# D-Robotics/hobot_stereonet

Hardware: AMD Instinct MI355X
Metric: stereo pairs/s at 1280x720 D=192 (ms/frame alongside) (higher is better)
Workload: dtype f16 (refinement-tower MFMA operands fp16 — 3x3 weights rounded per kernel so that every kernel's tap sum survives —, LeakyReLU applied after the fp16 rounding; low-resolution branch on 22-bit hi/lo split fp16 operands, 3 fp16 MFMAs per product in every 32-channel layer — profiles/r04_lowres_ablation

## Files before the change

hobot_stereonet_amd/csrc/sn_kernels.hpp:

```cpp
#pragma once
#include <hip/hip_runtime.h>
#include <stdint.h>

#include <type_traits>

#ifndef SN_X3S_FPK
#define SN_X3S_FPK 2
#endif
#ifndef SN_X3S_WAGPR
#define SN_X3S_WAGPR 1
#endif

namespace sn {

typedef float f32x16 __attribute__((ext_vector_type(16)));
typedef float f32x4 __attribute__((ext_vector_type(4)));

typedef _Float16 half8 __attribute__((ext_vector_type(8)));
typedef _Float16 half4 __attribute__((ext_vector_type(4)));

constexpr int kC = 32;
constexpr int kRefPad = 8;
constexpr float kSplitScale = 2048.0f;
constexpr float kSplitInv = 1.0f / 2048.0f;
// ... 1481 lines not shown
    if (NBUF == 3) {
      more = g0 + 3 < G;
      if (more) issue(g0 + 3, nimg_, ny0, nx0);
    } else {
      more = g0 + 2 < G;
      if (more) issue(g0 + 2, nimg_, ny0, nx0);
    }
    compute(lds + ((g0 + 1) % NBUF) * RING, std::integral_constant<int, 1>{}, acc0, acc1);
    if (RES) {
      if (more) wait_vmcnt<KW2>(); else wait_vmcnt<0>();
#pragma unroll
      for (int i = 0; i < 2 * T::NSTORE; ++i) asm volatile("" : "+v"(rres[i]));
    }
    const bool interior = y0 + T::TH <= g.H && x0 + T::TW <= g.W;
#pragma unroll
    for (int q = 0; q < 4; ++q) {
      char* oq = reinterpret_cast<char*>(out) + (tb + (unsigned)q * plane_b);
      char* oql = out_lo + (tb + (unsigned)q * plane_b);
#pragma unroll
      for (int s = 0; s < T::SPW; ++s) {
        half4 hh, hl;
#pragma unroll
        for (int e = 0; e < 4; ++e) {
          float v = acc0[s][4 * q + e] + acc1[s][4 * q + e] * kSplitInv;
          if (RES) {
            const uint2 rh = rres[RES ? 2 * (s * 4 + q) : 0], rl = rres[RES ? 2 * (s * 4 + q) + 1 : 0];
            const half4 vh = *reinterpret_cast<const half4*>(&rh);
            const half4 vl = *reinterpret_cast<const half4*>(&rl);
            v += (float)vh[e] + (float)vl[e] * kSplitInv;
          }
          if (lrelu) v = lrelu_fast(v);
          const _Float16 hi = (_Float16)v;
          hh[e] = hi;
          hl[e] = (_Float16)((v - (float)hi) * kSplitScale);
        }
        if (!interior) {
          const int seg = seg0 + s;
          const int y = y0 + seg / T::CSEG, x = x0 + (seg % T::CSEG) * 32 + j;
          if (!(y < g.H && x < g.W)) {
            hh = half4{(_Float16)0.f, (_Float16)0.f, (_Float16)0.f, (_Float16)0.f};
            hl = hh;
          }
        }
        *reinterpret_cast<half4*>(oq + io_voff[s]) = hh;
        *reinterpret_cast<half4*>(oql + io_voff[s]) = hl;
      }
    }
    img = nimg_;
    y0 = ny0;
    x0 = nx0;
  }
}

template <int TW_>
struct RefInTile {
  static constexpr int TH = 8, TW = TW_, CSEG = TW / 32;
  static constexpr int ROWS = TH + 2, COLS = TW + 8;
  static constexpr int BUF = ROWS * COLS;
  static constexpr int LDS_BYTES = 2 * BUF * 16;
  static constexpr int NUNIT = ROWS * (COLS / 4);
  static constexpr int SPW = TH * CSEG / 4;
};

template <bool SPLIT, bool PYR, int TW>
__global__ __launch_bounds__(256, 2) void k_refin_f16(const float* __restrict__ disp_low,
                                                   const void* __restrict__ img_src,
                                                   int hl, int wl, int H, int W, float inv_d, UpScale ups,
                                                   const uint4* __restrict__ wfrag,
                                                   const float* __restrict__ bias, uint4* __restrict__ out,
                                                   size_t lo_off_bytes, RefGeom g, int nimg, int al4) {
  using T = RefInTile<TW>;
  static_assert(T::NUNIT <= 256, "one staging unit per thread");
  extern __shared__ __attribute__((aligned(16))) uint4 s_px[];
  const int tid = threadIdx.x, lane = tid & 63;
  const int wave = __builtin_amdgcn_readfirstlane(tid >> 6);
  const int j = lane & 31, gk = lane >> 5;

  half8 wa[5], wb[5];
#pragma unroll
  for (int t = 0; t < 5; ++t) {
    const uint4 a = wfrag[(2 * t) * 64 + lane], b = wfrag[(2 * t + 1) * 64 + lane];
    wa[t] = *reinterpret_cast<const half8*>(&a);
    wb[t] = *reinterpret_cast<const half8*>(&b);
  }
  f32x16 bv;
#pragma unroll
  for (int r = 0; r < 16; ++r) bv[r] = bias[(r & 3) + 8 * (r >> 2) + 4 * gk];
  int koff[5];
#pragma unroll
  for (int t = 0; t < 5; ++t) {
    int tap = 2 * t + gk;
    tap = tap < 9 ? tap : 0;
    koff[t] = (tap / 3) * T::COLS + (tap % 3) + 3;
  }

  const int per_img = g.tiles_x * g.tiles_y;
  const int total = per_img * nimg;
  const int ur = tid / (T::COLS / 4), uq = tid - ur * (T::COLS / 4);
  const bool unit = tid < T::NUNIT;
  const int8_t* const in6 = reinterpret_cast<const int8_t*>(img_src);
  const float* const pyr = reinterpret_cast<const float*>(img_src);
  const bool x16 = ups.rs == 1.0f / 16.0f;
  uint32_t pimg[3];
  float pf[PYR ? 3 : 1][4];
  float pd[4];
  bool pval[4];
  auto fetch = [&](int tile) {
    if (g.rev) tile = total - 1 - tile;
    const int img = tile / per_img, rem = tile - img * per_img;
    const int ty = rem / g.tiles_x, tx = rem - ty * g.tiles_x;
    const int y = ty * T::TH - 1 + ur, x = tx * T::TW - 4 + 4 * uq;
    pimg[0] = pimg[1] = pimg[2] = 0;
#pragma unroll
    for (int k = 0; k < 4; ++k) {
      pd[k] = 0.f;
      pval[k] = false;
    }
// ... 23 lines not shown
      for (int k = 0; k < 4; ++k)
        if (pval[k]) pd[k] = upsample_map(dl, hl, wl, y, x + k, ups) * inv_d;
    }
    if (PYR) {
#pragma unroll
      for (int c = 0; c < 3; ++c) {
        const float* row = pyr + (((size_t)img * 3 + c) * g.H + y) * (size_t)g.W;
#pragma unroll
        for (int k = 0; k < 4; ++k) pf[PYR ? c : 0][k] = pval[k] ? row[x + k] : 0.f;
      }
    } else if (y < H) {
#pragma unroll
      for (int c = 0; c < 3; ++c) {
        const int8_t* row = in6 + (((size_t)img * 6 + c) * H + y) * (size_t)W;
        uint32_t v = 0;
        if (al4) {
          if (x >= 0 && x + 3 < W) v = *reinterpret_cast<const uint32_t*>(row + x);
        } else {
#pragma unroll
          for (int k = 0; k < 4; ++k)
            if ((unsigned)(x + k) < (unsigned)W) v |= (uint32_t)(uint8_t)row[x + k] << (8 * k);
        }
        pimg[c] = v;
      }
    }
  };
  auto commit = [&](uint4* buf) {
    if (!unit) return;
#pragma unroll
    for (int k = 0; k < 4; ++k) {
      half8 sl;
#pragma unroll
      for (int e = 0; e < 8; ++e) sl[e] = (_Float16)0.f;
      if (pval[k]) {
        const _Float16 dh = (_Float16)pd[k];
        sl[0] = dh;
        sl[4] = (_Float16)((pd[k] - (float)dh) * kSplitScale);
        if (PYR) {
#pragma unroll
          for (int c = 0; c < 3; ++c) {
            const float v = pf[PYR ? c : 0][k];
            const _Float16 vh = (_Float16)v;
            sl[1 + c] = vh;
            sl[5 + c] = (_Float16)((v - (float)vh) * kSplitScale);
          }
        } else {
#pragma unroll
          for (int c = 0; c < 3; ++c) sl[1 + c] = (_Float16)((float)(int8_t)(pimg[c] >> (8 * k)) * (1.0f / 128.0f));
        }
      }
      buf[ur * T::COLS + 4 * uq + k] = *reinterpret_cast<const uint4*>(&sl);
    }
  };

  int tile = blockIdx.x;
  if (tile >= total) return;
  fetch(tile);
  commit(s_px);
  __syncthreads();
  int cur = 0;
  const unsigned plane_b = (unsigned)g.Hs * (unsigned)g.Ws * 16u;
  unsigned io_voff[T::SPW];
#pragma unroll
  for (int s = 0; s < T::SPW; ++s) {
    const int seg = wave * T::SPW + s;
    io_voff[s] = ((unsigned)(seg / T::CSEG) * (unsigned)g.Ws + (unsigned)((seg % T::CSEG) * 32 + j)) * 16u + gk * 8u;
  }
  for (; tile < total; tile += gridDim.x) {
    const int nxt = tile + gridDim.x;
    if (nxt < total) fetch(nxt);
    const uint4* buf = s_px + cur * T::BUF;
    f32x16 acc0[T::SPW], acc1[T::SPW];
    f32x16 zero;
#pragma unroll
    for (int r = 0; r < 16; ++r) zero[r] = 0.f;
#pragma unroll
    for (int t = 0; t < 5; ++t) {
#pragma unroll
      for (int s = 0; s < T::SPW; ++s) {
        const int seg = wave * T::SPW + s;
        const int srow = seg / T::CSEG, scol = (seg % T::CSEG) * 32;
        const uint4 xv = buf[koff[t] + srow * T::COLS + scol + j];
        const half8 xb = *reinterpret_cast<const half8*>(&xv);
        acc0[s] = __builtin_amdgcn_mfma_f32_32x32x16_f16(wa[t], xb, t == 0 ? bv : acc0[s], 0, 0, 0);
        acc1[s] = __builtin_amdgcn_mfma_f32_32x32x16_f16(wb[t], xb, t == 0 ? zero : acc1[s], 0, 0, 0);
      }
    }
    {
      const int tile_m = g.rev ? total - 1 - tile : tile;
      const int img = tile_m / per_img, rem = tile_m - img * per_img;
      const int ty = rem / g.tiles_x, tx = rem - ty * g.tiles_x;
      const int y0 = ty * T::TH, x0 = tx * T::TW;
      const bool interior = y0 + T::TH <= g.H && x0 + T::TW <= g.W;
      const unsigned tb = (((unsigned)img * 4u * (unsigned)g.Hs + (unsigned)(y0 + kRefPad)) * (unsigned)g.Ws +
                           (unsigned)(x0 + kRefPad)) * 16u;
#pragma unroll
      for (int s = 0; s < T::SPW; ++s) {
#pragma unroll
        for (int q = 0; q < 4; ++q) {
          char* oq = reinterpret_cast<char*>(out) + (tb + (unsigned)q * plane_b);
          char* oql = oq + lo_off_bytes;
          half4 hh, hl4;
          if (SPLIT) {
#pragma unroll
            for (int e = 0; e < 4; ++e) {
              float v = acc0[s][4 * q + e] + acc1[s][4 * q + e] * kSplitInv;
              v = lrelu_fast(v);
              const _Float16 hi = (_Float16)v;
              hh[e] = hi;
              hl4[e] = (_Float16)((v - (float)hi) * kSplitScale);
            }
          } else {
            float v[4];
#pragma unroll
            for (int e = 0; e < 4; ++e) v[e] = acc0[s][4 * q + e] + acc1[s][4 * q + e] * kSplitInv;
            const uint2 pk{act_pack2_f16(v[0], v[1], (_Float16)kSlope), act_pack2_f16(v[2], v[3], (_Float16)kSlope)};
            hh = *reinterpret_cast<const half4*>(&pk);
          }
          bool ok = true;
          if (!interior) {
            const int seg = wave * T::SPW + s;
            ok = y0 + seg / T::CSEG < g.H && x0 + (seg % T::CSEG) * 32 + j < g.W;
          }
          if (ok) {
            *reinterpret_cast<half4*>(oq + io_voff[s]) = hh;
            if (SPLIT) *reinterpret_cast<half4*>(oql + io_voff[s]) = hl4;
          }
        }
      }
    }
    if (nxt < total) commit(s_px + (cur ^ 1) * T::BUF);
    lds_barrier();
    cur ^= 1;
  }
}

template <int TH_>
struct HeadTile {
  static constexpr int TH = TH_, TWO = 62;
  static constexpr int RP = TH + 2, CP = 64;
  static constexpr int NSEG = RP * 2, SPW = (NSEG + 3) / 4;
  static constexpr int PLANE = RP * CP;
  static constexpr int LDS_BYTES = 9 * PLANE * 4;
};

template <bool SPLIT, int TH>
__global__ __launch_bounds__(256) void k_head_final_f16(const uint4* __restrict__ xin, size_t lo_slots, RefGeom g,
                                                        const float* __restrict__ w,
                                                        float bias, const float* __restrict__ disp_low, int hl,
                                                        int wl, int H, int W, float dmax, float inv_q,
                                                        float* __restrict__ out_disp, int32_t* __restrict__ out_raw,
                                                        int tiles_x, int tiles_y, UpScale ups,
                                                        unsigned long long* __restrict__ stat) {
  using T = HeadTile<TH>;
  extern __shared__ __attribute__((aligned(16))) float s_p[];
  const int tid = threadIdx.x, lane = tid & 63;
  const int wave = __builtin_amdgcn_readfirstlane(tid >> 6);
  const int j = lane & 31, gh = lane >> 5;
  int t = blockIdx.x;
  const int tx = t % tiles_x;
  t /= tiles_x;
  const int ty = t % tiles_y, n = t / tiles_y;
  const int y0 = ty * T::TH, x0 = tx * T::TWO;

  const size_t plane_s = (size_t)g.Hs * g.Ws;
  const uint4* img = xin + (size_t)n * 4 * plane_s;
  uint4 xb[T::SPW][2], xl[SPLIT ? T::SPW : 1][2];
#pragma unroll
  for (int s = 0; s < T::SPW; ++s) {
    int seg = wave * T::SPW + s;
    seg = seg < T::NSEG ? seg : T::NSEG - 1;
    const int prow = seg >> 1, pcol = (seg & 1) * 32 + j;
    const size_t slot = (size_t)(y0 - 1 + prow + kRefPad) * g.Ws + (x0 - 1 + pcol + kRefPad);
#pragma unroll
    for (int kk = 0; kk < 2; ++kk) {
      xb[s][kk] = img[(size_t)(2 * kk + gh) * plane_s + slot];
      if (SPLIT) xl[s][kk] = img[(size_t)(2 * kk + gh) * plane_s + slot + lo_slots];
    }
  }
  half8 ah[2], al[2];
#pragma unroll
  for (int kk = 0; kk < 2; ++kk)
#pragma unroll
    for (int e = 0; e < 8; ++e) {
// ... 141 lines not shown
```

hobot_stereonet_amd/csrc/stereonet_hip.hip:

```cpp
#include <hip/hip_runtime.h>

#include <algorithm>

#include <atomic>
#include <chrono>
#include <cmath>
#include <condition_variable>
#include <cstdio>
#include <cstdlib>
#include <cstring>
#include <mutex>
#include <string>
#include <unordered_map>
#include <vector>

#ifndef SN_DIAGNOSTICS
#define SN_DIAGNOSTICS 0
#endif

#include "../../include/stereonet_hip.h"
#include "sn_internal.h"
#include "sn_kernels.hpp"
#include "sn_pointcloud.hpp"

// ... 110 lines not shown
  HeadLayer rout;
  RefGeom rg{};
  int Hk = 0, Wk = 0;
};

struct Slot {
  hipStream_t stream = nullptr;
  hipEvent_t ev0 = nullptr, ev1 = nullptr;
  Workspace ws;
  int8_t* pin_in = nullptr;
  int32_t* pin_raw = nullptr;
  float* pin_disp = nullptr;
  int32_t* user_raw = nullptr;
  float* user_disp = nullptr;
  uint64_t ticket = 0;
  hipGraphExec_t gexec[2][4][4] = {};
  int uses[2][4][4] = {};
  int mode_run = 0;
};

struct AutoCtl {
  sn_auto_state st{};
  bool calibrated = false;
  bool pending = false;
  int pending_mode = 0, pending_n = 0;
  double selfcheck_epe = -1.0, selfcheck_res = -1.0;
  double last_level[4] = {}, last_res = 0.0;
  int last_mode = 0;
  uint64_t calls = 0, pairs = 0, reruns = 0;
};

}

struct sn_handle {
  int device = 0;
  int W = 0, H = 0, D = 0, Wp = 0, Hp = 0, wl = 0, hl = 0, Dl = 0;
  int max_batch = 1, precision = SN_PREC_F16, task_num = 4, refine_chunk = 1, piece = 16;
  AutoCtl actl;
  std::mutex mu_cal;
  float* chk[2] = {nullptr, nullptr};
  hipEvent_t ev_stats = nullptr;
  int refine_chunk_x3 = 1;
  hipStream_t stream = nullptr;
  hipStream_t s_low = nullptr, s_tow[kMaxTowerStreams] = {};
  hipEvent_t ev_fork = nullptr, ev_join = nullptr, ev_tow_join[kMaxTowerStreams] = {}, ev_piece[kMaxPieceEvents] = {};
  bool overlap = true;
  int tower_streams = kMaxTowerStreams;
#if SN_DIAGNOSTICS
  unsigned ablate_x = 0;
#else
  static constexpr unsigned ablate_x = 0;
#endif
  bool tail_fuse = true;
  int fuse_mode = 4;
  unsigned* dump = nullptr;
  bool use_graphs = true;
  bool stream_prio = false;
  ConvLayer down[kNDown], fres[kNFeatRes][2], fout, agg[kNAgg];
  Down0F16 down0;
  Down01W down01;
  bool fold_down01 = false;
  HeadLayer aout;
  int levels = 1;
  Tower tw[kMaxLevels];
  int num_cu = 256;
  Workspace ws;
  std::vector<Slot> slots;
  std::mutex mu;
  std::condition_variable cv;
  uint64_t next_ticket = 1;
  bool profiling = false;
  hipEvent_t ev[8] = {};
  hipEvent_t ev_dom[2 * 6] = {};
  int dom_pairs = 0;
  float stage_ms[SN_STAGE_COUNT] = {};
  mutable std::string err;
  mutable std::mutex err_mu;
  struct PointCloud {
    std::mutex mu;
    hipStream_t stream = nullptr;
    hipEvent_t ev = nullptr;
    uint32_t* scratch = nullptr;
    size_t scratch_bytes = 0;
    void* dev[4] = {};
    size_t dev_bytes[4] = {};
    void* pin[2] = {};
    size_t pin_bytes[2] = {};
  } pc;
};

namespace {

void set_err(const sn_handle* h, const std::string& s) {
  if (h) {
    std::lock_guard<std::mutex> lk(h->err_mu);
    h->err = s;
  }
}
void set_err(std::nullptr_t, const std::string&) {}

template <class T>
hipError_t dalloc(T** p, size_t count) {
  return hipMalloc(reinterpret_cast<void**>(p), count * sizeof(T) + 256);
}

struct SnwHeader {
// ... 80 lines not shown
          const int co = lane & 31, c = ch * 16 + 8 * (lane >> 5) + e;
          const float w = wv(co, c, tap);
          const _Float16 hi = (_Float16)w;
          const size_t base = (((size_t)ch * taps + tap) * 2) * 64 * 8 + (size_t)lane * 8 + e;
          pk[base] = hi;
          pk[base + 64 * 8] = zero_lo ? (_Float16)0.f : (_Float16)((w - (float)hi) * kSplitScale);
        }
  HIP_TRY(h, dalloc(&out->wx3, pk.size() / 8));
  HIP_TRY(h, hipMemcpy(out->wx3, pk.data(), pk.size() * sizeof(_Float16), hipMemcpyHostToDevice));
  return SN_OK;
}

int upload_down0_f16(sn_handle* h, const HostLayer& l, Down0F16* out) {
  std::vector<_Float16> pk((size_t)8 * 2 * 64 * 8);
  for (int t = 0; t < 8; ++t)
    for (int lane = 0; lane < 64; ++lane)
      for (int e = 0; e < 8; ++e) {
        const int co = lane & 31, rho = 2 * t + (lane >> 5);
        const float w = (rho < 15 && e < 5) ? l.w[((size_t)co * 3 + rho / 5) * 25 + (rho % 5) * 5 + e] : 0.f;
        const _Float16 hi = (_Float16)w;
        const size_t base = ((size_t)(2 * t) * 64 + lane) * 8 + e;
        pk[base] = hi;
        pk[base + 64 * 8] = (_Float16)((w - (float)hi) * kSplitScale);
      }
  HIP_TRY(h, dalloc(&out->wfrag, pk.size() / 8));
  HIP_TRY(h, hipMemcpy(out->wfrag, pk.data(), pk.size() * sizeof(_Float16), hipMemcpyHostToDevice));
  return SN_OK;
}

int upload_refin_f16(sn_handle* h, const HostLayer& l, Down0F16* out) {
  std::vector<_Float16> pk((size_t)5 * 2 * 64 * 8, (_Float16)0.f);
  for (int t = 0; t < 5; ++t)
    for (int lane = 0; lane < 64; ++lane) {
      const int co = lane & 31, tap = 2 * t + (lane >> 5);
      if (tap >= 9) continue;
      _Float16* a = &pk[((size_t)(2 * t) * 64 + lane) * 8];
      _Float16* b = a + 64 * 8;
      for (int c = 0; c < 4; ++c) {
        const float w = l.w[((size_t)co * 4 + c) * 9 + tap];
        const _Float16 hi = (_Float16)w;
        a[c] = hi;
        b[c] = (_Float16)((w - (float)hi) * kSplitScale);
        b[4 + c] = hi;
      }
    }
  HIP_TRY(h, dalloc(&out->wfrag, pk.size() / 8));
  HIP_TRY(h, hipMemcpy(out->wfrag, pk.data(), pk.size() * sizeof(_Float16), hipMemcpyHostToDevice));
  return SN_OK;
}

template <int TW>
hipError_t launch_refin_f16_tw(hipStream_t st, const Down0F16& L, const float* bias, const float* disp_low,
                               const void* img_src, bool pyr, int hl, int wl, int H, int W, float inv_d, UpScale ups,
                               RefGeom g, int nimg, uint4* out, bool split, size_t lo_off_bytes, int num_cu) {
  using T = RefInTile<TW>;
  g.tiles_x = (g.W + TW - 1) / TW;
  g.tiles_y = (g.H + T::TH - 1) / T::TH;
  const int total = g.tiles_x * g.tiles_y * nimg;
  int blocks = 2 * num_cu;
  if (blocks > total) blocks = total;
  const int al4 = !pyr && (W % 4 == 0) && (reinterpret_cast<uintptr_t>(img_src) % 4 == 0);
#define SN_REFIN(S, P)                                                                                             \
  hipLaunchKernelGGL((k_refin_f16<S, P, TW>), dim3(blocks), dim3(256), T::LDS_BYTES, st, disp_low, img_src, hl, wl, H, \
                     W, inv_d, ups, L.wfrag, bias, out, lo_off_bytes, g, nimg, al4)
  if (split && pyr) SN_REFIN(true, true);
  else if (split) SN_REFIN(true, false);
  else if (pyr) SN_REFIN(false, true);
  else SN_REFIN(false, false);
#undef SN_REFIN
  return hipGetLastError();
}

hipError_t launch_refin_f16(hipStream_t st, const Down0F16& L, const float* bias, const float* disp_low,
                            const void* img_src, bool pyr, int hl, int wl, int H, int W, float inv_d, UpScale ups,
                            const RefGeom& g, int nimg, uint4* out, bool split, size_t lo_off_bytes, int num_cu) {
  return launch_refin_f16_tw<64>(st, L, bias, disp_low, img_src, pyr, hl, wl, H, W, inv_d, ups, g, nimg, out, split,
                                 lo_off_bytes, num_cu);
}

hipError_t launch_down0_f16(hipStream_t st, const Down0F16& L, const float* bias, const int8_t* in6, int H, int W,
                            int nimg, int Ho, int Wo, float* out, int num_cu, const SlotGeom* og = nullptr) {
  constexpr int TC = 32;
  using T = Down0Tile<TC>;
  const int tiles_x = (Wo + TC - 1) / TC, tiles_y = (Ho + T::TR - 1) / T::TR;
  const int total = tiles_x * tiles_y * nimg;
  int blocks = 2 * num_cu;
  if (blocks > total) blocks = total;
  const int al4 = (W % 4 == 0) && (reinterpret_cast<uintptr_t>(in6) % 4 == 0);
  hipLaunchKernelGGL((k_down0_f16<TC>), dim3(blocks), dim3(256), T::LDS_BYTES, st, in6, H, W, L.wfrag, bias, out, Ho, Wo,
                     tiles_x, tiles_y, nimg, 0, al4, og ? og->PH : Ho, og ? og->PW : Wo, og ? og->py : 0, og ? og->px : 0);
  return hipGetLastError();
}

template <class K>
hipError_t ensure_lds_attr(K kern, int bytes);

bool down01_enabled() {
  static const bool on = !(getenv("SN_DOWN01") != nullptr && atoi(getenv("SN_DOWN01")) == 0);
  return on;
}

int upload_down01(sn_handle* h, const HostLayer& l0, const HostLayer& l1, Down01W* out) {
  std::vector<double> weff, beff;
  compose_down01(l0.w, l0.b, l1.w, l1.b, weff, beff);
  std::vector<_Float16> pk;
  pack_down01(weff, pk);
  std::vector<float> bf(beff.begin(), beff.end());
  HIP_TRY(h, dalloc(&out->wfrag, pk.size() / 8));
  HIP_TRY(h, dalloc(&out->bias, bf.size()));
  HIP_TRY(h, hipMemcpy(out->wfrag, pk.data(), pk.size() * sizeof(_Float16), hipMemcpyHostToDevice));
  HIP_TRY(h, hipMemcpy(out->bias, bf.data(), bf.size() * sizeof(float), hipMemcpyHostToDevice));
  return SN_OK;
}

hipError_t launch_down01(hipStream_t st, const Down01W& L, const int8_t* in6, int H, int W, int nimg, int Ho, int Wo,
                         uint4* out, const SlotGeom& og, int num_cu) {
  using T = Down01;
  const bool w4 = (W % 4) == 0;
  hipError_t e = w4 ? ensure_lds_attr(k_down01_f16<true>, T::LDS_BYTES) : ensure_lds_attr(k_down01_f16<false>, T::LDS_BYTES);
  if (e != hipSuccess) return e;
  const int tiles_x = (Wo + T::TC - 1) / T::TC, tiles_y = (Ho + T::TR - 1) / T::TR;
  const int total = tiles_x * tiles_y * nimg;
  int blocks = num_cu / 8 * 8;
  while (blocks > 8 && blocks / 8 > (total + 7) / 8) blocks -= 8;
  if (w4)
    hipLaunchKernelGGL(k_down01_f16<true>, dim3(blocks), dim3(256), T::LDS_BYTES, st, in6, H, W,
                       L.wfrag + (size_t)T::INNER * T::NK * 2 * 64, L.bias + T::INNER * kC, out, Ho, Wo, tiles_x, tiles_y, nimg,
                       og.PH, og.PW, og.py, og.px);
  else
    hipLaunchKernelGGL(k_down01_f16<false>, dim3(blocks), dim3(256), T::LDS_BYTES, st, in6, H, W,
// ... 974 lines not shown
  static const int forced = getenv("SN_FIRST_PIECE") ? atoi(getenv("SN_FIRST_PIECE")) : 0;
  int m = ws.pb;
  if (h->precision == SN_PREC_FP32) m = ws.rb * ws.ns > 2 ? ws.rb * ws.ns : 2;
  if (forced > 0) m = forced;
  if (m > ws.pb) m = ws.pb;
  return m < n ? m : n;
}

int refine_level(sn_handle* h, Workspace& ws, hipStream_t st, const Tower& T, float* rx, float* rt, uint4* rx16,
                 uint4* rt16, const float* src, int sh, int sw, UpScale ups, const void* img_src, bool pyr, int H, int W,
                 float dnorm, float* od, int32_t* orw, unsigned* chunk_ctr, int c, int cap, bool pe, int mode,
                 unsigned long long* stat) {
  const int ncu = h->num_cu;
  const int tcu = ws.tower_cu > 0 ? ws.tower_cu : ncu;
  const int Hk = T.Hk, Wk = T.Wk;
  const float inv_q = (float)(1.0 / (kWireFactor * (double)kOutScale));
  if (mode == SN_PREC_FP32) {
    LoadRefineIn ld{src, reinterpret_cast<const int8_t*>(img_src), sh, sw, H, W, Hk, Wk, 1.0f / dnorm, ups,
                    pyr ? reinterpret_cast<const float*>(img_src) : nullptr};
    if (Hk * Wk <= 64 * 128)
      HIP_TRY(h, (launch_conv<3, 1, 1, 4, 4, 32>(st, T.rin, ld, c, Hk, Wk, rx, nullptr, true)));
    else
      HIP_TRY(h, (launch_conv<3, 1, 1, 4, 8, 64>(st, T.rin, ld, c, Hk, Wk, rx, nullptr, true)));
    if (pe) HIP_TRY(h, hipEventRecord(h->ev[4], st));
    for (int i = 0; i < kNRefRes; ++i) {
      HIP_TRY(h, conv3x3(st, T.rres[i][0], rx, c, Hk, Wk, kRefDil[i], rt, nullptr, true, ncu));
      HIP_TRY(h, conv3x3(st, T.rres[i][1], rt, c, Hk, Wk, kRefDil[i], rx, rx, true, ncu));
    }
    if (pe) HIP_TRY(h, hipEventRecord(h->ev[5], st));
    static const bool head_mfma = !(getenv("SN_HEAD_MFMA32") != nullptr && atoi(getenv("SN_HEAD_MFMA32")) == 0);
    if (head_mfma) {
      constexpr int TH = 14;
      using HT = HeadTile<TH>;
      const int tiles_x = (W + HT::TWO - 1) / HT::TWO, tiles_y = (H + TH - 1) / TH;
      hipLaunchKernelGGL(k_head_final_mfma32<TH>, dim3((unsigned)(tiles_x * tiles_y * c)), dim3(256), HT::LDS_BYTES, st, rx,
                         T.rout.w, T.rout.bias, src, sh, sw, Hk, Wk, H, W, dnorm, inv_q, od, orw, tiles_x, tiles_y, ups, stat);
    } else {
      dim3 grid((W + 63) / 64, (H + 3) / 4, c);
      hipLaunchKernelGGL(k_head_final, grid, dim3(256), 0, st, rx, T.rout.w, T.rout.bias, src, sh, sw, Hk, Wk, H, W, dnorm,
                         inv_q, od, orw, ups, stat);
    }
  } else {
    uint4* x16 = rx16;
    uint4* t16 = rt16;
    if (pe) h->dom_pairs = 0;
    static const int rev_env = getenv("SN_REV") ? atoi(getenv("SN_REV")) : 1;
    RefGeom g = T.rg;
    int launch_no = 0;
    auto flip = [&]() { g.rev = rev_env ? (launch_no++ & 1) : 0; };
    flip();
    const bool x3 = mode == SN_PREC_F16X3;
    const size_t lo_slots = ref16_slots(g, cap) + ref_slack(g);
    HIP_TRY(h, launch_refin_f16(st, T.refin, T.rin.bias, src, img_src, pyr, sh, sw, H, W, 1.0f / dnorm, ups, g, c, x16, x3,
                                lo_slots * 16, ncu));
    if (pe) HIP_TRY(h, hipEventRecord(h->ev[4], st));
    flip();
    const bool last_streamed = h->fuse_mode == 4 && stream_block_supports(kRefDil[kNRefRes - 1]);
    const bool tail = !x3 && last_streamed && h->tail_fuse && kRefDil[kNRefRes - 1] == 1 && ups.rs <= 0.5f;
    for (int i = 0; i < kNRefRes; ++i) {
      if (x3) {
        const bool dom = pe && stream_x3_supports(kRefDil[i]) && h->dom_pairs < 6;
        if (dom) HIP_TRY(h, hipEventRecord(h->ev_dom[2 * h->dom_pairs], st));
        HIP_TRY(h, ref_block_f16x3(st, T.rres16x3[i][0], T.rres16x3[i][1], g, tcu, kRefDil[i], &x16, &t16, lo_slots, c));
        if (dom) HIP_TRY(h, hipEventRecord(h->ev_dom[2 * h->dom_pairs++ + 1], st));
      } else if (tail && i == kNRefRes - 1) {
        if (pe) HIP_TRY(h, hipEventRecord(h->ev[5], st));
        StreamHeadArgs ha{T.rout.w, src, od, orw, T.rout.bias, dnorm, inv_q, sh, sw, H, W, ups, stat};
        HIP_TRY(h, ref_block_stream_tail(st, T.rres16[i][0], T.rres16[i][1], g, tcu, x16, c, h->dump, ha));
      } else {
        const bool dom = pe && h->fuse_mode == 4 && stream_block_supports(kRefDil[i]) && h->dom_pairs < 6;
        if (dom) HIP_TRY(h, hipEventRecord(h->ev_dom[2 * h->dom_pairs], st));
        HIP_TRY(h, ref_block_f16(st, T.rres16[i][0], T.rres16[i][1], g, tcu, kRefDil[i], &x16, &t16, c,
                                 chunk_ctr + 2 * i * kTileCtrStride, h->fuse_mode, h->dump, rev_env != 0));
        if (dom) HIP_TRY(h, hipEventRecord(h->ev_dom[2 * h->dom_pairs++ + 1], st));
      }
    }
    if (!tail) {
      if (pe) HIP_TRY(h, hipEventRecord(h->ev[5], st));
      HIP_TRY(h, launch_head_final_f16(st, x3, x16, lo_slots, g, T.rout.w, T.rout.bias, src, sh, sw, H, W, dnorm, inv_q, ups,
                                       od, orw, c, stat));
    }
  }
  HIP_TRY(h, hipGetLastError());
  return SN_OK;
}

inline int chunk_pairs(const sn_handle* h, const Workspace& ws, int mode, int lv = 0) {
  return (h->precision == SN_PREC_AUTO && mode == SN_PREC_F16X3) ? ws.rbk_x3[lv] : ws.rbk[lv];
}

inline int take_ctr_block(sn_handle* h, Workspace& ws, int* ctr_block, unsigned** out) {
  *out = nullptr;
  if (!ws.tile_ctr) return SN_OK;
  if (*ctr_block >= ws.n_chunks) {
    set_err(h, "internal: tile-queue pool exhausted");
    return SN_ERR_DEVICE;
  }
  *out = ws.tile_ctr + (size_t)(*ctr_block)++ * (kTileCtrBytes / sizeof(unsigned));
  return SN_OK;
}

int refine_coarse(sn_handle* h, Workspace& ws, hipStream_t st, int p0, int m, const int8_t* in6, int* ctr_block, int mode) {
  const size_t HW = (size_t)h->H * h->W;
  const int8_t* in_piece = in6 + (size_t)p0 * 6 * HW;
  for (int lv = 1; lv < h->levels; ++lv) {
    const Tower& T = h->tw[lv];
    const long total = (long)m * 3 * T.Hk * T.Wk;
// ... 469 lines not shown
    const double vol_elems = (double)pb * h->Dl * kC * h->hl * h->wl;
    double ref_bytes = 0;
    for (int lv = 0; lv < h->levels; ++lv) {
      const RefGeom& rg = h->tw[lv].rg;
      const double b = ((double)level_chunk_pairs(h->refine_chunk, pb, lv) * 4.0 * rg.Hs * rg.Ws + (double)ref_slack(rg) + (double)ref_front(rg)) * 16.0;
      if (b > ref_bytes) ref_bytes = b;
    }
    if (low_elems >= 4.0e9 || ref_bytes >= 4.0e9 || vol_elems >= 4.0e9) {
      delete h;
      return SN_ERR_ARG;
    }
  }
  int rc = check_device(h);
  auto fail = [&](int code) {
    create_fail(code, h->err.empty() ? "engine set-up" : h->err.c_str());
    sn_destroy(h);
    return code;
  };
  if (rc) return fail(rc);
  if (hipStreamCreateWithFlags(&h->stream, hipStreamNonBlocking) != hipSuccess) return fail(SN_ERR_DEVICE);
  for (auto& e : h->ev)
    if (hipEventCreate(&e) != hipSuccess) return fail(SN_ERR_DEVICE);
  for (auto& e : h->ev_dom)
    if (hipEventCreate(&e) != hipSuccess) return fail(SN_ERR_DEVICE);
  if (hipEventCreateWithFlags(&h->ev_stats, hipEventDisableTiming) != hipSuccess) return fail(SN_ERR_DEVICE);
  if (c.precision == SN_PREC_AUTO)
    for (auto& p : h->chk)
      if (dalloc(&p, (size_t)H * W) != hipSuccess) return fail(SN_ERR_NOMEM);
  int prio = 0;
  {
    int least = 0, greatest = 0;
    const char* e = getenv("SN_STREAM_PRIORITY");
    const bool want = (e && *e) ? atoi(e) == 1 : stream_prio == 1;
    if (want && hipDeviceGetStreamPriorityRange(&least, &greatest) == hipSuccess) prio = greatest;
  }
  h->stream_prio = prio != 0;
  auto mk_stream = [&](hipStream_t* st) {
    return prio != 0 ? hipStreamCreateWithPriority(st, hipStreamNonBlocking, prio) : hipStreamCreateWithFlags(st, hipStreamNonBlocking);
  };
  if (mk_stream(&h->s_low) != hipSuccess ||
      hipEventCreateWithFlags(&h->ev_fork, hipEventDisableTiming) != hipSuccess ||
      hipEventCreateWithFlags(&h->ev_join, hipEventDisableTiming) != hipSuccess)
    return fail(SN_ERR_DEVICE);
  for (int i = 0; i < kMaxTowerStreams; ++i)
    if (mk_stream(&h->s_tow[i]) != hipSuccess ||
        hipEventCreateWithFlags(&h->ev_tow_join[i], hipEventDisableTiming) != hipSuccess)
      return fail(SN_ERR_DEVICE);
  for (auto& e : h->ev_piece)
    if (hipEventCreateWithFlags(&e, hipEventDisableTiming) != hipSuccess) return fail(SN_ERR_DEVICE);
  h->overlap = getenv("SN_NO_OVERLAP") == nullptr;
  h->use_graphs = getenv("SN_NO_GRAPH") == nullptr;
  h->fuse_mode = fuse_env();
  h->tail_fuse = !(getenv("SN_TAIL_FUSE") != nullptr && atoi(getenv("SN_TAIL_FUSE")) == 0);
  if (hipMalloc(reinterpret_cast<void**>(&h->dump), 4096) != hipSuccess) return fail(SN_ERR_NOMEM);

  BlobWalker bw{blob.data()};
  const bool low_x3 = h->precision != SN_PREC_FP32;
  const unsigned abl_w = ablate_mask("SN_ABLATE_W");
#if SN_DIAGNOSTICS
  h->ablate_x = ablate_mask("SN_ABLATE_X");
#endif
  int feat_idx = 0;
  h->fold_down01 = low_x3 && down01_enabled();
  HostLayer hl_down0{};
  for (int i = 0; i < kNDown; ++i) {
    const HostLayer hl_ = bw.next(kC, i == 0 ? 3 : kC, 25);
    if ((rc = upload_conv2d(h, hl_, 4, &h->down[i]))) return fail(rc);
    if (low_x3 && i == 0 && (rc = upload_down0_f16(h, hl_, &h->down0))) return fail(rc);
    if (i == 0) hl_down0 = hl_;
    if (h->fold_down01 && i == 1 && (rc = upload_down01(h, hl_down0, hl_, &h->down01))) return fail(rc);
    if (low_x3 && i > 0 &&
        (rc = upload_x3(h, kC, [&](int co, int c, int tap) { return hl_.w[((size_t)co * kC + c) * 25 + tap]; },
                        &h->down[i], 25, (abl_w >> (kAblDown + i - 1)) & 1u)))
      return fail(rc);
  }
  auto up2d = [&](ConvLayer* L) -> int {
    const HostLayer hl_ = bw.next(kC, kC, 9);
    int r = upload_conv2d(h, hl_, 8, L);
    if (r || !low_x3) return r;
    const bool z = (abl_w >> (kAblFeat + feat_idx)) & 1u;
    ++feat_idx;
    return upload_x3(h, kC, [&](int co, int c, int tap) { return hl_.w[((size_t)co * kC + c) * 9 + tap]; }, L, 9, z);
  };
  for (int i = 0; i < kNFeatRes; ++i)
    for (int j = 0; j < 2; ++j)
      if ((rc = up2d(&h->fres[i][j]))) return fail(rc);
  if ((rc = up2d(&h->fout))) return fail(rc);
  for (int i = 0; i < kNAgg; ++i) {
    const HostLayer hl_ = bw.next(kC, kC, 27);
    if ((rc = upload_conv3d(h, hl_, &h->agg[i]))) return fail(rc);
    if (low_x3 && (rc = upload_x3(h, 96, [&](int co, int c, int tap) {
          return hl_.w[(((size_t)co * kC + (c & 31)) * 3 + (c >> 5)) * 9 + tap];
        }, &h->agg[i], 9, (abl_w >> (kAblAgg + i)) & 1u)))
      return fail(rc);
  }
  {
    const HostLayer hl_ = bw.next(1, kC, 27);
    if ((rc = upload_head(h, hl_, &h->aout))) return fail(rc);
    if (low_x3 && (rc = upload_agg_head_frag(h, hl_, &h->aout))) return fail(rc);
  }
  for (int lv = 0; lv < h->levels; ++lv) {
    Tower& T = h->tw[lv];
    {
      const HostLayer hl_ = bw.next(kC, 4, 9);
      if ((rc = upload_conv2d(h, hl_, 4, &T.rin))) return fail(rc);
      if (h->precision != SN_PREC_FP32 && (rc = upload_refin_f16(h, hl_, &T.refin))) return fail(rc);
// ... 789 lines not shown
  if (rc) return rc;
  const int Hp = (h_px + 15) / 16 * 16, Wp = (w + 15) / 16 * 16, Ho = Hp / 4, Wo = Wp / 4;
  Down01W L;
  const HostLayer l0{w0, b0, kC, 3, 25}, l1{w1, b1, kC, kC, 25};
  rc = upload_down01(h, l0, l1, &L);
  ds.track(L.wfrag);
  ds.track(L.bias);
  if (rc) return rc;
  int8_t* din = nullptr;
  uint4* dout = nullptr;
  const size_t nin = (size_t)6 * h_px * w, nout = (size_t)2 * kC * Ho * Wo;
  HIP_TRY(h, dalloc(&din, nin));
  ds.track(din);
  HIP_TRY(h, dalloc(&dout, nout / 4));
  ds.track(dout);
  HIP_TRY(h, hipMemcpy(din, in6, nin, hipMemcpyHostToDevice));
  HIP_TRY(h, launch_down01(h->stream, L, din, h_px, w, 2, Ho, Wo, dout, SlotGeom{Ho, Wo, 0, 0}, h->num_cu));
  HIP_TRY(h, hipStreamSynchronize(h->stream));
  std::vector<_Float16> hs(nout * 2);
  HIP_TRY(h, hipMemcpy(hs.data(), dout, nout * 4, hipMemcpyDeviceToHost));
  host_from_slots(hs, 2, Ho, Wo, out);
  return SN_OK;
}

int sn_dbg_refin(sn_handle* h, const float* disp_low, const int8_t* in6, int h_px, int w, int dmax, const float* wt,
                 const float* bias, int split, float* out) {
  DevScope ds;
  if (!h || !disp_low || !in6 || !wt || !bias || !out || h_px <= 0 || w <= 0 || dmax <= 0) return SN_ERR_ARG;
  int rc = check_device(h);
  if (rc) return rc;
  const int Hp = (h_px + 15) / 16 * 16, Wp = (w + 15) / 16 * 16, hl = Hp / 16, wl = Wp / 16;
  const RefGeom g = make_ref_geom(Hp, Wp);
  const size_t slots = ref16_slots(g, 1) + ref_slack(g);
  Down0F16 L;
  HostLayer hl_{wt, bias, kC, 4, 9};
  if ((rc = upload_refin_f16(h, hl_, &L))) return rc;
  ds.track(L.wfrag);
  float *ddl = nullptr, *dbias = nullptr;
  int8_t* din = nullptr;
  uint4* dout = nullptr;
  HIP_TRY(h, dalloc(&ddl, (size_t)hl * wl));
  ds.track(ddl);
  HIP_TRY(h, dalloc(&dbias, kC));
  ds.track(dbias);
  HIP_TRY(h, dalloc(&din, (size_t)6 * h_px * w));
  ds.track(din);
  HIP_TRY(h, dalloc(&dout, 2 * slots));
  ds.track(dout);
  HIP_TRY(h, hipMemcpy(ddl, disp_low, (size_t)hl * wl * 4, hipMemcpyHostToDevice));
  HIP_TRY(h, hipMemcpy(dbias, bias, kC * 4, hipMemcpyHostToDevice));
  HIP_TRY(h, hipMemcpy(din, in6, (size_t)6 * h_px * w, hipMemcpyHostToDevice));
  HIP_TRY(h, memset_now(dout, 0, 2 * slots * 16));
  HIP_TRY(h, launch_refin_f16(h->stream, L, dbias, ddl, din, false, hl, wl, h_px, w, 1.0f / (float)dmax,
                              UpScale{1.0f / 16.0f, 16.0f}, g, 1, dout, split != 0, slots * 16, h->num_cu));
  HIP_TRY(h, hipStreamSynchronize(h->stream));
  std::vector<_Float16> hout(2 * slots * 8);
  HIP_TRY(h, hipMemcpy(hout.data(), dout, 2 * slots * 16, hipMemcpyDeviceToHost));
  for (int c = 0; c < kC; ++c)
    for (int y = 0; y < Hp; ++y)
      for (int x = 0; x < Wp; ++x) {
        const size_t i = ((((size_t)(c >> 3)) * g.Hs + y + kRefPad) * g.Ws + x + kRefPad) * 8 + (c & 7);
        float v = (float)hout[i];
        if (split) v += (float)hout[i + slots * 8] * kSplitInv;
        out[((size_t)c * Hp + y) * Wp + x] = v;
      }
  for (int c = 0; c < 4; ++c)
    for (int y = 0; y < g.Hs; ++y)
      for (int x = 0; x < g.Ws; ++x) {
        if (y >= kRefPad && y < kRefPad + Hp && x >= kRefPad && x < kRefPad + Wp) continue;
        for (int e = 0; e < 8; ++e)
          if ((float)hout[(((size_t)c * g.Hs + y) * g.Ws + x) * 8 + e] != 0.f) {
            set_err(h, "ref.in wrote into the zero border");
            return SN_ERR_DEVICE;
          }
      }
  return SN_OK;
}

int sn_dbg_conv3d(sn_handle* h, const float* in, int d, int h_px, int w, const float* wt, const float* bias,
                  int lrelu, float* out) {
  DevScope ds;
  if (!h || !in || !wt || !bias || !out || d <= 0) return SN_ERR_ARG;
  int rc = check_device(h);
  if (rc) return rc;
  const bool x3 = (lrelu & 2) != 0, slots = (lrelu & 4) != 0, dma = (lrelu & 8) != 0;
  lrelu &= 1;
  if (slots != x3 || (dma && !slots)) return SN_ERR_ARG;
  ConvLayer L;
  HostLayer hl{wt, bias, kC, kC, 27};
  if ((rc = upload_conv3d(h, hl, &L))) return rc;
  ds.track(L.bias); ds.track(L.wpk); ds.track(L.wx3);
  if (x3 && (rc = upload_x3(h, 96, [&](int co, int c, int tap) {
        return wt[(((size_t)co * kC + (c & 31)) * 3 + (c >> 5)) * 9 + tap];
      }, &L)))
    return rc;
  ds.track(L.wx3);
  const size_t plane = (size_t)h_px * w, n = (size_t)kC * d * plane;
  std::vector<float> tmp(n);
  for (int ci = 0; ci < kC; ++ci)
    for (int z = 0; z < d; ++z)
      memcpy(&tmp[((size_t)z * kC + ci) * plane], &in[((size_t)ci * d + z) * plane], plane * 4);
  float *din = nullptr, *dout = nullptr;
  HIP_TRY(h, dalloc(&din, n));
  ds.track(din);
  HIP_TRY(h, dalloc(&dout, n));
  ds.track(dout);
  if (slots) {
// ... 547 lines not shown
```

Measured before the change: 3082.

## Defer refinement-input staging math until after MFMAs and write border zeros in-kernel

Adds a second variant of the refinement-input kernel for the non-pyramid, 16x-upscale, 4-aligned case. This variant prefetches only the four raw low-res disparity taps and the int8 pixels into registers, then performs the bilinear upsampling and fp16 split conversion while committing to LDS after the MFMA work. It also lets out-of-image lanes write zeros into the padded border instead of branching. The aim is to lower register pressure and latency in the prefetch and keep the stores uniform, at the cost of recomputing tile geometry and a larger LDS staging buffer. The old path remains available through SN_REFIN_V1.

New measurement: 3094 (median of 6 runs). Within noise of the previous version (+0.4%).

```diff
diff --git a/hobot_stereonet_amd/csrc/sn_kernels.hpp b/hobot_stereonet_amd/csrc/sn_kernels.hpp
--- a/hobot_stereonet_amd/csrc/sn_kernels.hpp
+++ b/hobot_stereonet_amd/csrc/sn_kernels.hpp
@@ -1557,6 +1557,26 @@
   }
 }
 
+template <bool SPLIT>
+__device__ __forceinline__ void refin_act(const f32x16& acc0, const f32x16& acc1, int q, half4& hh, half4& hl4) {
+  if (SPLIT) {
+#pragma unroll
+    for (int e = 0; e < 4; ++e) {
+      float v = acc0[4 * q + e] + acc1[4 * q + e] * kSplitInv;
+      v = lrelu_fast(v);
+      const _Float16 hi = (_Float16)v;
+      hh[e] = hi;
+      hl4[e] = (_Float16)((v - (float)hi) * kSplitScale);
+    }
+  } else {
+    float v[4];
+#pragma unroll
+    for (int e = 0; e < 4; ++e) v[e] = acc0[4 * q + e] + acc1[4 * q + e] * kSplitInv;
+    const uint2 pk{act_pack2_f16(v[0], v[1], (_Float16)kSlope), act_pack2_f16(v[2], v[3], (_Float16)kSlope)};
+    hh = *reinterpret_cast<const half4*>(&pk);
+  }
+}
+
 template <int TW_>
 struct RefInTile {
   static constexpr int TH = 8, TW = TW_, CSEG = TW / 32;
@@ -1565,9 +1585,12 @@
   static constexpr int LDS_BYTES = 2 * BUF * 16;
   static constexpr int NUNIT = ROWS * (COLS / 4);
   static constexpr int SPW = TH * CSEG / 4;
+  static constexpr int ROWS2 = (256 + COLS / 4 - 1) / (COLS / 4);
+  static constexpr int BUF2 = ROWS2 * COLS;
+  static constexpr int LDS_BYTES2 = 2 * BUF2 * 16;
 };
 
-template <bool SPLIT, bool PYR, int TW>
+template <bool SPLIT, bool PYR, int TW, bool V1>
 __global__ __launch_bounds__(256, 2) void k_refin_f16(const float* __restrict__ disp_low,
                                                    const void* __restrict__ img_src,
                                                    int hl, int wl, int H, int W, float inv_d, UpScale ups,
@@ -1697,11 +1720,90 @@
       buf[ur * T::COLS + 4 * uq + k] = *reinterpret_cast<const uint4*>(&sl);
     }
   };
-
+  static_assert(V1 || !PYR, "the deferred form reads the int8 source");
+  struct UnitGeom {
+    int img, y, x, y0, x0, y1, x1;
+    float ly;
+    bool row, img_ok;
+  };
+  auto unit_geom = [&](int tile) {
+    UnitGeom u;
+    if (g.rev) tile = total - 1 - tile;
+    u.img = tile / per_img;
+    const int rem = tile - u.img * per_img;
+    const int ty = rem / g.tiles_x, tx = rem - ty * g.tiles_x;
+    u.y = ty * T::TH - 1 + ur;
+    u.x = tx * T::TW - 4 + 4 * uq;
+    u.row = unit && (unsigned)u.y < (unsigned)g.H;
+    const int ya = u.row ? u.y : 0, xa = (u.x >= 0 && u.x < g.W) ? u.x : 0;
+    float sy = ((float)ya + 0.5f) * ups.rs - 0.5f;
+    sy = sy < 0.f ? 0.f : sy;
+    float sx0 = ((float)xa + 0.5f) * ups.rs - 0.5f;
+    sx0 = sx0 < 0.f ? 0.f : sx0;
+    u.y0 = (int)sy;
+    u.x0 = (int)sx0;
+    u.y1 = u.y0 < hl - 1 ? u.y0 + 1 : u.y0;
+    u.x1 = u.x0 < wl - 1 ? u.x0 + 1 : u.x0;
+    u.ly = sy - (float)u.y0;
+    u.img_ok = u.row && u.y < H && u.x >= 0 && u.x + 3 < W;
+    return u;
+  };
+  float ta[4];
+  auto fetch2 = [&](int tile) {
+    const UnitGeom u = unit_geom(tile);
+    const float* dl = disp_low + (size_t)u.img * hl * wl;
+    ta[0] = dl[u.y0 * wl + u.x0];
+    ta[1] = dl[u.y0 * wl + u.x1];
+    ta[2] = dl[u.y1 * wl + u.x0];
+    ta[3] = dl[u.y1 * wl + u.x1];
+    const int yi = u.img_ok ? u.y : 0, xi = u.img_ok ? u.x : 0;
+#pragma unroll
+    for (int c = 0; c < 3; ++c)
+      pimg[c] = *reinterpret_cast<const uint32_t*>(in6 + (((size_t)u.img * 6 + c) * H + yi) * (size_t)W + xi);
+  };
+  auto commit2 = [&](int tile, uint4* buf) {
+    const UnitGeom u = unit_geom(tile);
+    const float ly = u.ly, hy = 1.0f - ly;
+    const float a00 = ta[0], a01 = ta[1], a10 = ta[2], a11 = ta[3];
+#pragma unroll
+    for (int c = 0; c < 3; ++c) pimg[c] = u.img_ok ? pimg[c] : 0u;
+#pragma unroll
+    for (int k = 0; k < 4; ++k) {
+      float sx = ((float)(u.x + k) + 0.5f) * ups.rs - 0.5f;
+      sx = sx < 0.f ? 0.f : sx;
+      const float lx = sx - (float)u.x0, hx = 1.0f - lx;
+      const bool in = u.row && (unsigned)(u.x + k) < (unsigned)g.W;
+      float d;
+      {
+#pragma clang fp contract(off)
+        const float b = __builtin_fmaf(hx, a10, lx * a11);
+        const float v = k == 0 ? __builtin_fmaf(hy, __builtin_fmaf(hx, a00, lx * a01), ly * b)
+                               : hy * __builtin_fmaf(lx, a01, hx * a00) + ly * b;
+        d = in ? v * ups.mul * inv_d : 0.f;
+      }
+      half8 sl;
+      const _Float16 dh = (_Float16)d;
+      sl[0] = dh;
+      sl[4] = (_Float16)((d - (float)dh) * kSplitScale);
+#pragma unroll
+      for (int c = 0; c < 3; ++c) sl[1 + c] = (_Float16)((float)(int8_t)(pimg[c] >> (8 * k)) * (1.0f / 128.0f));
+      sl[5] = sl[6] = sl[7] = (_Float16)0.f;
+      uint4 w = *reinterpret_cast<const uint4*>(&sl);
+      if (!in) w = uint4{0u, 0u, 0u, 0u};
+      buf[ur * T::COLS + 4 * uq + k] = w;
+    }
+  };
+
+  constexpr int BUFS = V1 ? T::BUF : T::BUF2;
   int tile = blockIdx.x;
   if (tile >= total) return;
-  fetch(tile);
-  commit(s_px);
+  if (V1) {
+    fetch(tile);
+    commit(s_px);
+  } else {
+    fetch2(tile);
+    commit2(tile, s_px);
+  }
   __syncthreads();
   int cur = 0;
   const unsigned plane_b = (unsigned)g.Hs * (unsigned)g.Ws * 16u;
@@ -1713,8 +1815,12 @@
   }
   for (; tile < total; tile += gridDim.x) {
     const int nxt = tile + gridDim.x;
-    if (nxt < total) fetch(nxt);
-    const uint4* buf = s_px + cur * T::BUF;
+    if (V1) {
+      if (nxt < total) fetch(nxt);
+    } else {
+      fetch2(nxt < total ? nxt : tile);
+    }
+    const uint4* buf = s_px + cur * BUFS;
     f32x16 acc0[T::SPW], acc1[T::SPW];
     f32x16 zero;
 #pragma unroll
@@ -1731,12 +1837,12 @@
         acc1[s] = __builtin_amdgcn_mfma_f32_32x32x16_f16(wb[t], xb, t == 0 ? zero : acc1[s], 0, 0, 0);
       }
     }
-    {
-      const int tile_m = g.rev ? total - 1 - tile : tile;
-      const int img = tile_m / per_img, rem = tile_m - img * per_img;
-      const int ty = rem / g.tiles_x, tx = rem - ty * g.tiles_x;
-      const int y0 = ty * T::TH, x0 = tx * T::TW;
-      const bool interior = y0 + T::TH <= g.H && x0 + T::TW <= g.W;
+    const int tile_m = g.rev ? total - 1 - tile : tile;
+    const int img = tile_m / per_img, rem = tile_m - img * per_img;
+    const int ty = rem / g.tiles_x, tx = rem - ty * g.tiles_x;
+    const int y0 = ty * T::TH, x0 = tx * T::TW;
+    const bool interior = y0 + T::TH <= g.H && x0 + T::TW <= g.W;
+    if (V1) {
       const unsigned tb = (((unsigned)img * 4u * (unsigned)g.Hs + (unsigned)(y0 + kRefPad)) * (unsigned)g.Ws +
                            (unsigned)(x0 + kRefPad)) * 16u;
 #pragma unroll
@@ -1746,22 +1852,7 @@
           char* oq = reinterpret_cast<char*>(out) + (tb + (unsigned)q * plane_b);
           char* oql = oq + lo_off_bytes;
           half4 hh, hl4;
-          if (SPLIT) {
-#pragma unroll
-            for (int e = 0; e < 4; ++e) {
-              float v = acc0[s][4 * q + e] + acc1[s][4 * q + e] * kSplitInv;
-              v = lrelu_fast(v);
-              const _Float16 hi = (_Float16)v;
-              hh[e] = hi;
-              hl4[e] = (_Float16)((v - (float)hi) * kSplitScale);
-            }
-          } else {
-            float v[4];
-#pragma unroll
-            for (int e = 0; e < 4; ++e) v[e] = acc0[s][4 * q + e] + acc1[s][4 * q + e] * kSplitInv;
-            const uint2 pk{act_pack2_f16(v[0], v[1], (_Float16)kSlope), act_pack2_f16(v[2], v[3], (_Float16)kSlope)};
-            hh = *reinterpret_cast<const half4*>(&pk);
-          }
+          refin_act<SPLIT>(acc0[s], acc1[s], q, hh, hl4);
           bool ok = true;
           if (!interior) {
             const int seg = wave * T::SPW + s;
@@ -1773,8 +1864,34 @@
           }
         }
       }
-    }
-    if (nxt < total) commit(s_px + (cur ^ 1) * T::BUF);
+      if (nxt < total) commit(s_px + (cur ^ 1) * T::BUF);
+    } else {
+      const unsigned ib = (unsigned)img * 4u * (unsigned)g.Hs * (unsigned)g.Ws * 16u;
+      const unsigned rb = (unsigned)(y0 + kRefPad) * (unsigned)g.Ws * 16u;
+      const unsigned cb = (unsigned)(x0 + kRefPad) * 16u;
+#pragma unroll
+      for (int s = 0; s < T::SPW; ++s) {
+        const int seg = wave * T::SPW + s;
+        const int srow = seg / T::CSEG;
+        const bool ok = interior || (y0 + srow < g.H && x0 + (seg % T::CSEG) * 32 + j < g.W);
+        const unsigned voff =
+            rb + (ok ? cb + io_voff[s] : ((unsigned)srow * (unsigned)g.Ws + (unsigned)(j & 7)) * 16u + gk * 8u);
+#pragma unroll
+        for (int q = 0; q < 4; ++q) {
+          char* oq = reinterpret_cast<char*>(out) + (ib + (unsigned)q * plane_b);
+          char* oql = oq + lo_off_bytes;
+          half4 hh, hl4;
+          refin_act<SPLIT>(acc0[s], acc1[s], q, hh, hl4);
+          if (!ok) {
+            hh = half4{(_Float16)0.f, (_Float16)0.f, (_Float16)0.f, (_Float16)0.f};
+            hl4 = hh;
+          }
+          *reinterpret_cast<half4*>(oq + voff) = hh;
+          if (SPLIT) *reinterpret_cast<half4*>(oql + voff) = hl4;
+        }
+      }
+      commit2(nxt < total ? nxt : tile, s_px + (cur ^ 1) * BUFS);
+    }
     lds_barrier();
     cur ^= 1;
   }
diff --git a/hobot_stereonet_amd/csrc/stereonet_hip.hip b/hobot_stereonet_amd/csrc/stereonet_hip.hip
--- a/hobot_stereonet_amd/csrc/stereonet_hip.hip
+++ b/hobot_stereonet_amd/csrc/stereonet_hip.hip
@@ -186,6 +186,7 @@
   static constexpr unsigned ablate_x = 0;
 #endif
   bool tail_fuse = true;
+  bool refin_v1 = false;
   int fuse_mode = 4;
   unsigned* dump = nullptr;
   bool use_graphs = true;
@@ -372,7 +373,8 @@
 template <int TW>
 hipError_t launch_refin_f16_tw(hipStream_t st, const Down0F16& L, const float* bias, const float* disp_low,
                                const void* img_src, bool pyr, int hl, int wl, int H, int W, float inv_d, UpScale ups,
-                               RefGeom g, int nimg, uint4* out, bool split, size_t lo_off_bytes, int num_cu) {
+                               RefGeom g, int nimg, uint4* out, bool split, size_t lo_off_bytes, int num_cu,
+                               bool v1) {
   using T = RefInTile<TW>;
   g.tiles_x = (g.W + TW - 1) / TW;
   g.tiles_y = (g.H + T::TH - 1) / T::TH;
@@ -380,22 +382,26 @@
   int blocks = 2 * num_cu;
   if (blocks > total) blocks = total;
   const int al4 = !pyr && (W % 4 == 0) && (reinterpret_cast<uintptr_t>(img_src) % 4 == 0);
-#define SN_REFIN(S, P)                                                                                             \
-  hipLaunchKernelGGL((k_refin_f16<S, P, TW>), dim3(blocks), dim3(256), T::LDS_BYTES, st, disp_low, img_src, hl, wl, H, \
-                     W, inv_d, ups, L.wfrag, bias, out, lo_off_bytes, g, nimg, al4)
-  if (split && pyr) SN_REFIN(true, true);
-  else if (split) SN_REFIN(true, false);
-  else if (pyr) SN_REFIN(false, true);
-  else SN_REFIN(false, false);
+#define SN_REFIN(S, P, V)                                                                                          \
+  hipLaunchKernelGGL((k_refin_f16<S, P, TW, V>), dim3(blocks), dim3(256), V ? T::LDS_BYTES : T::LDS_BYTES2, st, \
+                     disp_low, img_src, hl, wl, H, W, inv_d, ups, L.wfrag, bias, out, lo_off_bytes, g, nimg, al4)
+  const bool deferred = !v1 && !pyr && al4 && ups.rs == 1.0f / 16.0f;
+  if (split && pyr) SN_REFIN(true, true, true);
+  else if (pyr) SN_REFIN(false, true, true);
+  else if (split && deferred) SN_REFIN(true, false, false);
+  else if (split) SN_REFIN(true, false, true);
+  else if (deferred) SN_REFIN(false, false, false);
+  else SN_REFIN(false, false, true);
 #undef SN_REFIN
   return hipGetLastError();
 }
 
 hipError_t launch_refin_f16(hipStream_t st, const Down0F16& L, const float* bias, const float* disp_low,
                             const void* img_src, bool pyr, int hl, int wl, int H, int W, float inv_d, UpScale ups,
-                            const RefGeom& g, int nimg, uint4* out, bool split, size_t lo_off_bytes, int num_cu) {
+                            const RefGeom& g, int nimg, uint4* out, bool split, size_t lo_off_bytes, int num_cu,
+                            bool v1) {
   return launch_refin_f16_tw<64>(st, L, bias, disp_low, img_src, pyr, hl, wl, H, W, inv_d, ups, g, nimg, out, split,
-                                 lo_off_bytes, num_cu);
+                                 lo_off_bytes, num_cu, v1);
 }
 
 hipError_t launch_down0_f16(hipStream_t st, const Down0F16& L, const float* bias, const int8_t* in6, int H, int W,
@@ -1476,7 +1482,7 @@
     const bool x3 = mode == SN_PREC_F16X3;
     const size_t lo_slots = ref16_slots(g, cap) + ref_slack(g);
     HIP_TRY(h, launch_refin_f16(st, T.refin, T.rin.bias, src, img_src, pyr, sh, sw, H, W, 1.0f / dnorm, ups, g, c, x16, x3,
-                                lo_slots * 16, ncu));
+                                lo_slots * 16, ncu, h->refin_v1));
     if (pe) HIP_TRY(h, hipEventRecord(h->ev[4], st));
     flip();
     const bool last_streamed = h->fuse_mode == 4 && stream_block_supports(kRefDil[kNRefRes - 1]);
@@ -2052,6 +2058,7 @@
   h->use_graphs = getenv("SN_NO_GRAPH") == nullptr;
   h->fuse_mode = fuse_env();
   h->tail_fuse = !(getenv("SN_TAIL_FUSE") != nullptr && atoi(getenv("SN_TAIL_FUSE")) == 0);
+  h->refin_v1 = getenv("SN_REFIN_V1") != nullptr && atoi(getenv("SN_REFIN_V1")) != 0;
   if (hipMalloc(reinterpret_cast<void**>(&h->dump), 4096) != hipSuccess) return fail(SN_ERR_NOMEM);
 
   BlobWalker bw{blob.data()};
@@ -2947,7 +2954,8 @@
   HIP_TRY(h, hipMemcpy(din, in6, (size_t)6 * h_px * w, hipMemcpyHostToDevice));
   HIP_TRY(h, memset_now(dout, 0, 2 * slots * 16));
   HIP_TRY(h, launch_refin_f16(h->stream, L, dbias, ddl, din, false, hl, wl, h_px, w, 1.0f / (float)dmax,
-                              UpScale{1.0f / 16.0f, 16.0f}, g, 1, dout, split != 0, slots * 16, h->num_cu));
+                              UpScale{1.0f / 16.0f, 16.0f}, g, 1, dout, split != 0, slots * 16, h->num_cu,
+                              h->refin_v1));
   HIP_TRY(h, hipStreamSynchronize(h->stream));
   std::vector<_Float16> hout(2 * slots * 8);
   HIP_TRY(h, hipMemcpy(hout.data(), dout, 2 * slots * 16, hipMemcpyDeviceToHost));
```
